# Boese0601/MagicDance

Measured on NVIDIA H100. Metric: denoise-steps/sec @512x512 50-step DDIM, higher is better.
Workload: dtype f16

## Files before the change

include/magicdance_b200.h:

```cpp
#ifndef MAGICDANCE_B200_H_
#define MAGICDANCE_B200_H_

#include <stdint.h>

#ifdef __cplusplus
extern "C" {
#endif

#define MDB_OK 0
#define MDB_ERR_INVALID (-1)
#define MDB_ERR_CUDA (-2)
#define MDB_ERR_UNSUPPORTED (-3)

#define MDB_ABI_VERSION 2

typedef void* mdb_stream_t;

int mdb_abi_version(void);
const char* mdb_last_error(void);
int mdb_device_check(void);
int64_t mdb_launch_count(void);
int64_t mdb_abi_struct_bytes(int32_t which);

#define MDB_TUNE_GEMM_PAIR_MIN_TILES 1
#define MDB_TUNE_ATTN40_2Q_MIN_CTAS 3
#define MDB_TUNE_GEMM_BN80_BELOW 4
int mdb_set_tuning(int32_t key, int32_t value);
int32_t mdb_get_tuning(int32_t key);

#define MDB_EPI_NONE 0
#define MDB_EPI_GEGLU 1

typedef struct mdb_gemm_desc {
  const void* a;
  int64_t lda;
  const void* a2;
  int64_t lda2;
  int32_t k1;
  int32_t conv;
  int32_t nb, h, w, c;
  const void* b;
  int64_t ldb;
  void* d;
  int64_t ldd;
  const float* bias;
  int64_t bias_batch_stride;
  int32_t rows_per_batch;
  int32_t epilogue;
  const void* residual;
  int64_t ldr;
  int32_t m, n, k;
  int32_t splits;
  float* splitk_ws;
  const float* ln_u;
  float ln_eps;
} mdb_gemm_desc;

int mdb_gemm_f16(const mdb_gemm_desc* desc, mdb_stream_t stream);

#define MDB_DTYPE_F16 0
#define MDB_DTYPE_F32 1

typedef struct mdb_gemm_bwd_desc {
  mdb_gemm_desc fwd;
  const void* dd; int64_t lddd;
  void* da; int64_t ldda; int32_t da_dtype; int32_t da_accumulate;
  void* da2; int64_t ldda2; int32_t da2_dtype; int32_t da2_accumulate;
  void* db; int64_t lddb; int32_t db_dtype; int32_t db_accumulate;
  float* dbias; int32_t dbias_accumulate;
  int32_t splits;
  float* ws;
} mdb_gemm_bwd_desc;

int mdb_gemm_bwd_f16(const mdb_gemm_bwd_desc* desc, mdb_stream_t stream);
int64_t mdb_gemm_bwd_ws_floats(const mdb_gemm_bwd_desc* desc);

typedef struct mdb_attn_desc {
  const void* q; int64_t ldq;
  const void* k0; int64_t ldk0; const void* vt0; int64_t ldvt0; int32_t n0; int32_t kv0_batches; int32_t ldv0_batch;
  const void* k1; int64_t ldk1; const void* vt1; int64_t ldvt1; int32_t n1; int32_t kv1_batches; int32_t ldv1_batch;
  void* out; int64_t ldo;
  int32_t batch, heads, d, nq;
  int32_t bank_batches;
  float scale;
} mdb_attn_desc;

int mdb_attention_f16(const mdb_attn_desc* desc, mdb_stream_t stream);

int mdb_attention_lse_f16(const mdb_attn_desc* desc, float* lse, mdb_stream_t stream);

typedef struct mdb_attn_bwd_desc {
  mdb_attn_desc fwd;
  const void* dout; int64_t lddout;
  const float* lse;
  void* dq; int64_t lddq;
  void* dk0; int64_t lddk0; void* dvt0; int64_t lddvt0;
  void* dk1; int64_t lddk1; void* dvt1; int64_t lddvt1;
  float* ws;
} mdb_attn_bwd_desc;

int mdb_attention_bwd_f16(const mdb_attn_bwd_desc* desc, mdb_stream_t stream);
int64_t mdb_attention_bwd_ws_floats(int32_t batch, int32_t heads, int32_t nq);

int mdb_groupnorm_f16(const void* x1, int32_t c1, const void* x2, int32_t c2, const float* gamma, const float* beta,
                      void* y, float* ws, int32_t batch, int32_t hw, float eps, int32_t silu, int32_t mode,
                      mdb_stream_t stream);
int64_t mdb_groupnorm_ws_floats(int32_t c, int32_t batch, int32_t hw);

int mdb_layernorm_f16(const void* x, const float* gamma, const float* beta, void* y, int64_t rows, int32_t c,
// ... 67 lines not shown
```

magicdance_b200/_lib.py:

```python
from __future__ import annotations

import ctypes as C
import os

from . import build as _build

c_void_p, c_int32, c_int64, c_float = C.c_void_p, C.c_int32, C.c_int64, C.c_float


class GemmDesc(C.Structure):
    _fields_ = [
        ("a", c_void_p), ("lda", c_int64), ("a2", c_void_p), ("lda2", c_int64),
        ("k1", c_int32), ("conv", c_int32), ("nb", c_int32), ("h", c_int32), ("w", c_int32), ("c", c_int32),
        ("b", c_void_p), ("ldb", c_int64), ("d", c_void_p), ("ldd", c_int64),
        ("bias", c_void_p), ("bias_batch_stride", c_int64), ("rows_per_batch", c_int32), ("epilogue", c_int32),
        ("residual", c_void_p), ("ldr", c_int64),
        ("m", c_int32), ("n", c_int32), ("k", c_int32), ("splits", c_int32), ("splitk_ws", c_void_p),
        ("ln_u", c_void_p), ("ln_eps", c_float),
    ]


class AttnDesc(C.Structure):
    _fields_ = [
        ("q", c_void_p), ("ldq", c_int64),
# ... 20 lines not shown


class GemmBwdDesc(C.Structure):
    _fields_ = [
        ("fwd", GemmDesc),
        ("dd", c_void_p), ("lddd", c_int64),
        ("da", c_void_p), ("ldda", c_int64), ("da_dtype", c_int32), ("da_accumulate", c_int32),
        ("da2", c_void_p), ("ldda2", c_int64), ("da2_dtype", c_int32), ("da2_accumulate", c_int32),
        ("db", c_void_p), ("lddb", c_int64), ("db_dtype", c_int32), ("db_accumulate", c_int32),
        ("dbias", c_void_p), ("dbias_accumulate", c_int32),
        ("splits", c_int32),
        ("ws", c_void_p),
    ]


class GroupNormBwdDesc(C.Structure):
    _fields_ = [
        ("x1", c_void_p), ("x2", c_void_p), ("c1", c_int32), ("c2", c_int32),
        ("gamma", c_void_p), ("beta", c_void_p),
        ("dy", c_void_p),
        ("batch", c_int32), ("hw", c_int32), ("eps", c_float), ("silu", c_int32),
        ("dx1", c_void_p), ("dx1_dtype", c_int32), ("dx1_accumulate", c_int32),
        ("dx2", c_void_p), ("dx2_dtype", c_int32), ("dx2_accumulate", c_int32),
        ("dgamma", c_void_p), ("dbeta", c_void_p), ("dgamma_accumulate", c_int32), ("dbeta_accumulate", c_int32),
        ("ws", c_void_p),
    ]


class LayerNormBwdDesc(C.Structure):
    _fields_ = [
        ("x", c_void_p), ("gamma", c_void_p), ("dy", c_void_p),
        ("rows", c_int64), ("c", c_int32), ("eps", c_float),
        ("dx", c_void_p), ("dx_dtype", c_int32), ("dx_accumulate", c_int32),
        ("dgamma", c_void_p), ("dbeta", c_void_p), ("dgamma_accumulate", c_int32), ("dbeta_accumulate", c_int32),
        ("ws", c_void_p),
    ]


SIGNATURES = {
    "mdb_abi_version": (c_int32, []),
    "mdb_last_error": (C.c_char_p, []),
    "mdb_device_check": (c_int32, []),
    "mdb_launch_count": (c_int64, []),
    "mdb_abi_struct_bytes": (c_int64, [c_int32]),
    "mdb_set_tuning": (c_int32, [c_int32, c_int32]),
    "mdb_get_tuning": (c_int32, [c_int32]),
    "mdb_gemm_f16": (c_int32, [C.POINTER(GemmDesc), c_void_p]),
    "mdb_gemm_bwd_f16": (c_int32, [C.POINTER(GemmBwdDesc), c_void_p]),
    "mdb_gemm_bwd_ws_floats": (c_int64, [C.POINTER(GemmBwdDesc)]),
    "mdb_attention_f16": (c_int32, [C.POINTER(AttnDesc), c_void_p]),
    "mdb_attention_lse_f16": (c_int32, [C.POINTER(AttnDesc), c_void_p, c_void_p]),
    "mdb_attention_bwd_f16": (c_int32, [C.POINTER(AttnBwdDesc), c_void_p]),
    "mdb_attention_bwd_ws_floats": (c_int64, [c_int32, c_int32, c_int32]),
    "mdb_groupnorm_f16": (c_int32, [c_void_p, c_int32, c_void_p, c_int32, c_void_p, c_void_p, c_void_p, c_void_p,
                                    c_int32, c_int32, c_float, c_int32, c_int32, c_void_p]),
    "mdb_groupnorm_ws_floats": (c_int64, [c_int32, c_int32, c_int32]),
    "mdb_layernorm_f16": (c_int32, [c_void_p, c_void_p, c_void_p, c_void_p, c_int64, c_int32, c_float, c_void_p]),
    "mdb_groupnorm_bwd_f16": (c_int32, [C.POINTER(GroupNormBwdDesc), c_void_p]),
    "mdb_groupnorm_bwd_ws_floats": (c_int64, [C.POINTER(GroupNormBwdDesc)]),
    "mdb_layernorm_bwd_f16": (c_int32, [C.POINTER(LayerNormBwdDesc), c_void_p]),
    "mdb_layernorm_bwd_ws_floats": (c_int64, [C.POINTER(LayerNormBwdDesc)]),
    "mdb_geglu_f16": (c_int32, [c_void_p, c_int64, c_void_p, c_int64, c_int64, c_int32, c_void_p]),
    "mdb_geglu_bwd_f16": (c_int32, [c_void_p, c_int64, c_void_p, c_int64, c_void_p, c_int64, c_int64, c_int32,
                                    c_void_p]),
    "mdb_conv3x3_direct_f16": (c_int32, [c_void_p, c_void_p, c_void_p, c_void_p, c_void_p, c_int32, c_int32, c_int32,
                                         c_int32, c_int32, c_int32, c_int32, c_void_p]),
    "mdb_im2col3x3_f16": (c_int32, [c_void_p, c_void_p, c_int32, c_int32, c_int32, c_int32, c_int32, c_void_p]),
    "mdb_im2col3x3_br_f16": (c_int32, [c_void_p, c_void_p, c_int32, c_int32, c_int32, c_int32, c_int32, c_void_p]),
    "mdb_upsample2x_f16": (c_int32, [c_void_p, c_void_p, c_int32, c_int32, c_int32, c_int32, c_void_p]),
    "mdb_add_f16": (c_int32, [c_void_p, c_void_p, c_void_p, c_int64, c_int32, c_int32, c_void_p]),
    "mdb_timestep_embedding_f32": (c_int32, [c_void_p, c_int32, c_void_p, c_int32, c_int32, c_void_p]),
    "mdb_skinny_linear_f32": (c_int32, [c_void_p, c_void_p, c_void_p, c_void_p, c_int32, c_int32, c_int32, c_int32,
                                        c_int32, c_void_p]),
    "mdb_nchw_f32_to_nhwc_f16": (c_int32, [c_void_p, c_void_p, c_int32, c_int32, c_int32, c_int32, c_int32, c_void_p]),
    "mdb_nhwc_f16_to_nchw_f32": (c_int32, [c_void_p, c_void_p, c_int32, c_int32, c_int32, c_int32, c_void_p]),
    "mdb_softmax_rows_f16": (c_int32, [c_void_p, c_int64, c_int32, c_int32, c_float, c_void_p]),
    "mdb_cfg_ddim_update_f32": (c_int32, [c_void_p, c_void_p, c_void_p, c_void_p, c_void_p, c_void_p, c_int64,
                                          c_void_p, c_int32, c_void_p]),
}

_lib = None
ABI_VERSION = 2
TUNE_GEMM_PAIR_MIN_TILES, TUNE_ATTN40_2Q_MIN_CTAS, TUNE_GEMM_BN80_BELOW = 1, 3, 4


def library_path() -> str:
    return os.environ.get("MAGICDANCE_B200_LIB", _build.LIB_PATH)


def load():
    global _lib
    if _lib is not None:
        return _lib
    path = library_path()
    if not os.path.isfile(path):
        raise RuntimeError(
            f"magicdance_b200: kernel library {path} is missing — run `python -m magicdance_b200.build` "
            "(there is no CPU/PyTorch fallback for the hot path)")
    if path == _build.LIB_PATH and os.path.isdir(_build.CSRC) and not _build.is_fresh():
        raise RuntimeError(f"magicdance_b200: {path} was not built from the sources in {_build.CSRC} "
                           "(stamp mismatch) — run `python -m magicdance_b200.build`")
    lib = C.CDLL(path)
    for name, (res, args) in SIGNATURES.items():
        fn = getattr(lib, name)
        fn.restype = res
        fn.argtypes = args
    if lib.mdb_abi_version() != ABI_VERSION:
        raise RuntimeError(f"magicdance_b200: ABI version mismatch ({lib.mdb_abi_version()} != {ABI_VERSION}); "
                           "rebuild the library")
    for which, mirror in ((0, GemmDesc), (1, AttnDesc), (2, AttnBwdDesc), (3, GemmBwdDesc), (4, GroupNormBwdDesc),
                          (5, LayerNormBwdDesc)):
        if lib.mdb_abi_struct_bytes(which) != C.sizeof(mirror):
            raise RuntimeError(f"magicdance_b200: {mirror.__name__} mirrors {C.sizeof(mirror)} bytes, the library's "
                               f"struct has {lib.mdb_abi_struct_bytes(which)}: the binding and the library disagree")
    _lib = lib
    return lib


def check(rc: int, what: str):
    if rc != 0:
        msg = load().mdb_last_error().decode(errors="replace")
        raise RuntimeError(f"magicdance_b200.{what} failed (code {rc}): {msg}")
```

magicdance_b200/csrc/attention.cu:

```cuda
#include <stdlib.h>

#include <type_traits>

#include "common.cuh"

namespace mdb {

constexpr int kBQ = 128;

template <int D, int BKV, int STAGES>
struct AttnCfg {
  static constexpr int kDkChunks = (D + 63) / 64;
  static constexpr int kDV = (D + 15) / 16 * 16;
  static constexpr int kKSteps = kDV / 16;
  static constexpr int kQBytes = kDkChunks * kBQ * 128;
  static constexpr int kKBytes = kDkChunks * BKV * 128;
  static constexpr int kVBytes = kDV * 128;
  static constexpr int kStageBytes = kKBytes + kVBytes;
  static constexpr int kSmem = kQBytes + STAGES * kStageBytes + 1024;
  static_assert(BKV == 64, "one 128-byte swizzle row of keys per V^T tile");
  static_assert(kVBytes % 1024 == 0 && kKBytes % 1024 == 0, "stage tiles start on swizzle-atom boundaries");
};

struct AttnKParams {
// ... 92 lines not shown
      }
      wgmma_commit();
      wgmma_wait<0>();
      wgmma_fence_regs(sc);

      if (valid < BKV) {
#pragma unroll
        for (int i = 0; i < BKV / 2; ++i)
          if (8 * (i >> 2) + cq + (i & 1) >= valid) sc[i] = -INFINITY;
      }
      float mx[2] = {-INFINITY, -INFINITY};
#pragma unroll
      for (int i = 0; i < BKV / 2; ++i) mx[(i >> 1) & 1] = fmaxf(mx[(i >> 1) & 1], sc[i]);
      float alpha[2], neg_m[2];
#pragma unroll
      for (int h = 0; h < 2; ++h) {
        mx[h] = fmaxf(mx[h], __shfl_xor_sync(0xffffffffu, mx[h], 1));
        mx[h] = fmaxf(mx[h], __shfl_xor_sync(0xffffffffu, mx[h], 2));
        const float m_new = fmaxf(m_run[h], mx[h] * p.scale_log2);
        alpha[h] = ex2_approx(m_run[h] - m_new);
        m_run[h] = m_new;
        neg_m[h] = -m_new;
      }
      float ls[2] = {0.f, 0.f};
      uint32_t pa[BKV / 16][4];
#pragma unroll
      for (int i = 0; i < BKV / 2; i += 2) {
        const int h = (i >> 1) & 1;
        const float e0 = ex2_approx(fmaf(sc[i], p.scale_log2, neg_m[h]));
        const float e1 = ex2_approx(fmaf(sc[i + 1], p.scale_log2, neg_m[h]));
        ls[h] += e0 + e1;
        pa[i >> 3][(i >> 1) & 3] = pack_half2(e0, e1);
      }
#pragma unroll
      for (int h = 0; h < 2; ++h) l_run[h] = fmaf(l_run[h], alpha[h], ls[h]);
#pragma unroll
      for (int i = 0; i < C::kDV / 2; ++i) o[i] *= alpha[(i >> 1) & 1];

      wgmma_fence();
#pragma unroll
      for (int kk = 0; kk < BKV / 16; ++kk)
        wgmma_rs<C::kDV>(o, pa[kk], wgmma_desc_k_sw128(v_addr) + 2 * kk, 1u);
      wgmma_commit();
      wgmma_wait<0>();
      wgmma_fence_regs(o);
      mbar_arrive(&kv_empty[s]);
    }

    float inv_l[2], l_row[2];
#pragma unroll
    for (int h = 0; h < 2; ++h) {
      float l = l_run[h];
      l += __shfl_xor_sync(0xffffffffu, l, 1);
      l += __shfl_xor_sync(0xffffffffu, l, 2);
      inv_l[h] = 1.0f / l;
      l_row[h] = l;
    }
    const int r = wg * 64 + (warp & 3) * 16 + (lane >> 2);
    if constexpr (LSE) {
      if ((lane & 3) == 0) {
#pragma unroll
        for (int h = 0; h < 2; ++h) {
          const int q = q0 + r + 8 * h;
          if (q < p.nq)
            p.lse[(static_cast<long long>(b) * gridDim.y + head) * p.nq + q] =
                (m_run[h] + log2f(l_row[h])) * 0.6931471805599453f;
        }
      }
    }
#pragma unroll
    for (int h = 0; h < 2; ++h) {
      const int q = q0 + r + 8 * h;
      if (q < p.nq) {
        __half* op = p.out + (static_cast<long long>(b) * p.nq + q) * p.ldo + head * D + cq;
#pragma unroll
        for (int c8 = 0; c8 < D / 8; ++c8)
          *reinterpret_cast<uint32_t*>(op + 8 * c8) =
              pack_half2(o[4 * c8 + 2 * h] * inv_l[h], o[4 * c8 + 2 * h + 1] * inv_l[h]);
      }
    }
  }
}

static int g_attn40_2q_min_ctas = 512;
int get_attn_tuning() { return g_attn40_2q_min_ctas; }
void set_attn_tuning(int v) { g_attn40_2q_min_ctas = v; }

template <int D, int BKV, int STAGES, int MINB, bool LSE = false, typename P>
static int launch_attn(const P& kp, dim3 grid, cudaStream_t st) {
  using C = AttnCfg<D, BKV, STAGES>;
  static_assert(MINB == 1 || C::kSmem <= 113 * 1024, "two CTAs per SM must fit");
  constexpr auto kern = attn_wg_kernel<D, BKV, STAGES, MINB, LSE>;
  if (int rc = set_max_dyn_smem<kern>(C::kSmem)) return rc;
  MDB_CHECK_CUDA(launch_pdl(kern, grid, dim3(kWsThreads), C::kSmem, st, kp));
  count_launch();
  return MDB_OK;
}

template <int D, int BKV>
static int build_and_launch(const mdb_attn_desc* a, float* lse, cudaStream_t st) {
  constexpr int kDV = AttnCfg<D, BKV, 1>::kDV;
  AttnKParams kp;
  memset(&kp, 0, sizeof(kp));
  const int hd = a->heads * a->d;
  int rc;
  if ((rc = tmap_heads(&kp.tmQ, a->q, a->d, a->heads, (uint64_t)a->batch * a->nq, a->ldq, kBQ))) return rc;
  auto mk_kv = [&](const void* k, long long ldk, const void* vt, long long ldvt, int n, int nb, int ldvb,
                   CUtensorMap* tk, CUtensorMap* tv) -> int {
    int r = tmap_heads(tk, k, a->d, a->heads, (uint64_t)nb * n, ldk, BKV);
    if (r) return r;
    return tmap_vt(tv, vt, n, nb, ldvb, hd, ldvt, kDV);
  };
  if ((rc = mk_kv(a->k0, a->ldk0, a->vt0, a->ldvt0, a->n0, a->kv0_batches, a->ldv0_batch, &kp.tmK0, &kp.tmV0))) return rc;
  if (a->n1 > 0) {
    if ((rc = mk_kv(a->k1, a->ldk1, a->vt1, a->ldvt1, a->n1, a->kv1_batches, a->ldv1_batch, &kp.tmK1, &kp.tmV1)))
      return rc;
  }
  kp.out = static_cast<__half*>(a->out);
  kp.ldo = a->ldo;
  kp.nq = a->nq;
  kp.n0 = a->n0;
  kp.n1 = a->n1;
  kp.kv0_batches = a->kv0_batches;
  kp.kv1_batches = a->kv1_batches;
  kp.bank_batches = a->n1 > 0 ? a->bank_batches : 0;
  kp.scale_log2 = a->scale * 1.4426950408889634f;
  dim3 grid((a->nq + kBQ - 1) / kBQ, a->heads, a->batch);
  if (lse != nullptr) {
    AttnLseKParams lp;
    memset(&lp, 0, sizeof(lp));
    static_cast<AttnKParams&>(lp) = kp;
    lp.lse = lse;
    if constexpr (D == 40) {
      const long long ctas = (long long)grid.x * grid.y * grid.z;
      if (ctas >= (long long)g_attn40_2q_min_ctas) return launch_attn<D, BKV, 3, 2, true>(lp, grid, st);
    }
    return launch_attn<D, BKV, (D == 160 ? 2 : 4), 1, true>(lp, grid, st);
  }
  if constexpr (D == 40) {
    const long long ctas = (long long)grid.x * grid.y * grid.z;
    if (ctas >= (long long)g_attn40_2q_min_ctas) return launch_attn<D, BKV, 3, 2>(kp, grid, st);
  }
  return launch_attn<D, BKV, (D == 160 ? 2 : 4), 1>(kp, grid, st);
}

static int attention_entry(const mdb_attn_desc* a, float* lse, cudaStream_t st) {
  switch (a->d) {
    case 40:
      return build_and_launch<40, 64>(a, lse, st);
    case 80:
      return build_and_launch<80, 64>(a, lse, st);
    case 160:
      return build_and_launch<160, 64>(a, lse, st);
    default:
      set_error("mdb_attention_f16: head dim %d not supported (40, 80, 160)", a->d);
      return MDB_ERR_UNSUPPORTED;
  }
}

int attention_check_desc(const mdb_attn_desc* a) {
  MDB_REQUIRE(a != nullptr, "mdb_attention_f16: null descriptor");
  MDB_REQUIRE(a->q && a->k0 && a->vt0 && a->out, "mdb_attention_f16: null operand");
  MDB_REQUIRE(a->batch > 0 && a->heads > 0 && a->nq > 0 && a->n0 > 0 && a->n1 >= 0,
              "mdb_attention_f16: bad shape");
  MDB_REQUIRE(a->n1 == 0 || (a->k1 && a->vt1), "mdb_attention_f16: n1 > 0 needs k1/vt1");
  MDB_REQUIRE(a->kv0_batches == 1 || a->kv0_batches == a->batch, "mdb_attention_f16: kv0_batches must be 1 or batch");
  MDB_REQUIRE(a->n1 == 0 || a->kv1_batches == 1 || a->kv1_batches >= a->bank_batches,
              "mdb_attention_f16: kv1_batches must be 1 or cover bank_batches");
  MDB_REQUIRE(a->ldv0_batch >= a->n0 && a->ldv0_batch % 8 == 0, "mdb_attention_f16: ldv0_batch must be >= n0 and %% 8");
  MDB_REQUIRE(a->n1 == 0 || (a->ldv1_batch >= a->n1 && a->ldv1_batch % 8 == 0),
              "mdb_attention_f16: ldv1_batch must be >= n1 and %% 8");
  MDB_REQUIRE(a->ldo % 8 == 0 && (reinterpret_cast<uintptr_t>(a->out) & 15) == 0, "mdb_attention_f16: out alignment");
  return MDB_OK;
}

}

using namespace mdb;

extern "C" int mdb_attention_f16(const mdb_attn_desc* a, mdb_stream_t stream) {
  const int rc = attention_check_desc(a);
  if (rc) return rc;
  return attention_entry(a, nullptr, static_cast<cudaStream_t>(stream));
}

extern "C" int mdb_attention_lse_f16(const mdb_attn_desc* a, float* lse, mdb_stream_t stream) {
  const int rc = attention_check_desc(a);
  if (rc) return rc;
  MDB_REQUIRE(lse != nullptr, "mdb_attention_lse_f16: null lse");
  return attention_entry(a, lse, static_cast<cudaStream_t>(stream));
}
```

magicdance_b200/csrc/common.cuh:

```cuda
#pragma once

#include <cuda.h>
#include <cuda_fp16.h>
#include <cuda_runtime.h>
#include <cudaTypedefs.h>
#include <stdint.h>
#include <stdio.h>
#include <string.h>

#include "../../include/magicdance_b200.h"
#include "wgmma.cuh"

namespace mdb {

void set_error(const char* fmt, ...);

#define MDB_CHECK_CUDA(expr)                                                                     \
  do {                                                                                           \
    cudaError_t _e = (expr);                                                                     \
    if (_e != cudaSuccess) {                                                                     \
      mdb::set_error("%s:%d: %s failed: %s", __FILE__, __LINE__, #expr, cudaGetErrorString(_e)); \
      return MDB_ERR_CUDA;                                                                       \
    }                                                                                            \
  } while (0)

#define MDB_REQUIRE(cond, ...)      \
  do {                              \
    if (!(cond)) {                  \
      mdb::set_error(__VA_ARGS__);  \
      return MDB_ERR_INVALID;       \
    }                               \
  } while (0)

void count_launch(int n = 1);
int get_gemm_tuning(int key);
void set_gemm_tuning(int key, int value);
int get_attn_tuning();
void set_attn_tuning(int v);

constexpr int kNumSms = 132;

int tmap_rows(CUtensorMap* out, const void* base, uint64_t inner, uint64_t rows, long long ld, uint32_t box_inner,
              uint32_t box_rows);
int tmap_heads(CUtensorMap* out, const void* base, int d, int heads, uint64_t tokens, long long ld,
               uint32_t box_tokens);
int tmap_vt(CUtensorMap* out, const void* base, int n, int nb, long long ldvb, int rows, long long ldvt,
            uint32_t box_rows);
int tmap_nhwc(CUtensorMap* out, const void* base, int c, int w, int h, int nb, long long ld, const uint32_t box[4],
              int cs);

enum { kBoxOk, kBoxWideRows, kBoxRowsPerTile, kBoxImagesPerTile, kBoxTooLarge };
int pixel_box(int ho, int wo, int cs, int rows, bool fwd, uint32_t box[4]);

#ifdef __CUDACC__

bool pdl_enabled();
template <typename... KArgs, typename... Args>
inline cudaError_t launch_pdl_cluster2(void (*kernel)(KArgs...), dim3 grid, dim3 block, size_t smem,
                                       cudaStream_t stream, unsigned cluster_x, unsigned cluster_z, Args&&... args) {
  cudaLaunchConfig_t cfg;
  memset(&cfg, 0, sizeof(cfg));
  cfg.gridDim = grid;
  cfg.blockDim = block;
  cfg.dynamicSmemBytes = smem;
  cfg.stream = stream;
  cudaLaunchAttribute attr[2];
  int n = 0;
  if (cluster_z > 1 || cluster_x > 1) {
    attr[n].id = cudaLaunchAttributeClusterDimension;
    attr[n].val.clusterDim.x = cluster_x;
    attr[n].val.clusterDim.y = 1;
    attr[n].val.clusterDim.z = cluster_z;
    ++n;
  }
  if (pdl_enabled()) {
    attr[n].id = cudaLaunchAttributeProgrammaticStreamSerialization;
    attr[n].val.programmaticStreamSerializationAllowed = 1;
    ++n;
  }
  cfg.attrs = attr;
  cfg.numAttrs = n;
  return cudaLaunchKernelEx(&cfg, kernel, static_cast<KArgs>(args)...);
}
template <typename... KArgs, typename... Args>
inline cudaError_t launch_pdl_cluster(void (*kernel)(KArgs...), dim3 grid, dim3 block, size_t smem,
                                      cudaStream_t stream, unsigned cluster_z, Args&&... args) {
  return launch_pdl_cluster2(kernel, grid, block, smem, stream, 1u, cluster_z, static_cast<Args&&>(args)...);
}
template <typename... KArgs, typename... Args>
inline cudaError_t launch_pdl(void (*kernel)(KArgs...), dim3 grid, dim3 block, size_t smem, cudaStream_t stream,
                              Args&&... args) {
  return launch_pdl_cluster2(kernel, grid, block, smem, stream, 1u, 1u, static_cast<Args&&>(args)...);
}
template <auto Kernel>
inline int set_max_dyn_smem(int bytes) {
  static bool done = false;
  if (!done) {
    MDB_CHECK_CUDA(cudaFuncSetAttribute(Kernel, cudaFuncAttributeMaxDynamicSharedMemorySize, bytes));
    done = true;
  }
  return MDB_OK;
}

__device__ __forceinline__ uint32_t smem_u32(const void* p) {
  return static_cast<uint32_t>(__cvta_generic_to_shared(p));
}

__device__ __forceinline__ bool elect_one() {
  uint32_t pred = 0;
  asm volatile(
      "{\n\t.reg .pred P;\n\t"
      "elect.sync _|P, 0xffffffff;\n\t"
      "selp.u32 %0, 1, 0, P;\n\t}"
      : "=r"(pred));
  return pred != 0;
}

__device__ __forceinline__ void pdl_launch_dependents() { asm volatile("griddepcontrol.launch_dependents;" ::: "memory"); }
__device__ __forceinline__ void pdl_wait() { asm volatile("griddepcontrol.wait;" ::: "memory"); }

__device__ __forceinline__ void mbar_init(uint64_t* bar, uint32_t count) {
// ... 48 lines not shown
  const int s = it % S;
  mbar_wait(&full[s], (it / S) & 1);
  return s;
}

__device__ __forceinline__ void tma_prefetch_desc(const CUtensorMap* m) {
  asm volatile("prefetch.tensormap [%0];" ::"l"(reinterpret_cast<uint64_t>(m)) : "memory");
}
__device__ __forceinline__ void tma_load_2d(void* dst, const CUtensorMap* m, uint64_t* bar, int c0, int c1) {
  asm volatile(
      "cp.async.bulk.tensor.2d.shared::cluster.global.tile.mbarrier::complete_tx::bytes [%0], [%1, {%3, %4}], [%2];"
      ::"r"(smem_u32(dst)), "l"(reinterpret_cast<uint64_t>(m)), "r"(smem_u32(bar)), "r"(c0), "r"(c1)
      : "memory");
}
__device__ __forceinline__ void tma_load_3d(void* dst, const CUtensorMap* m, uint64_t* bar, int c0, int c1, int c2) {
  asm volatile(
      "cp.async.bulk.tensor.3d.shared::cluster.global.tile.mbarrier::complete_tx::bytes [%0], [%1, {%3, %4, %5}], [%2];"
      ::"r"(smem_u32(dst)), "l"(reinterpret_cast<uint64_t>(m)), "r"(smem_u32(bar)), "r"(c0), "r"(c1), "r"(c2)
      : "memory");
}
__device__ __forceinline__ void tma_load_4d(void* dst, const CUtensorMap* m, uint64_t* bar, int c0, int c1, int c2,
                                            int c3) {
  asm volatile(
      "cp.async.bulk.tensor.4d.shared::cluster.global.tile.mbarrier::complete_tx::bytes [%0], [%1, {%3, %4, %5, %6}], [%2];"
      ::"r"(smem_u32(dst)), "l"(reinterpret_cast<uint64_t>(m)), "r"(smem_u32(bar)), "r"(c0), "r"(c1), "r"(c2), "r"(c3)
      : "memory");
}

__device__ __forceinline__ uint32_t cluster_ctarank() {
  uint32_t r;
  asm volatile("mov.u32 %0, %%cluster_ctarank;" : "=r"(r));
  return r;
}
__device__ __forceinline__ void cluster_sync_all() {
  asm volatile("barrier.cluster.arrive.release.aligned;" ::: "memory");
  asm volatile("barrier.cluster.wait.acquire.aligned;" ::: "memory");
}
__device__ __forceinline__ uint32_t dsmem_map(uint32_t local_smem_addr, uint32_t rank) {
  uint32_t a;
  asm volatile("mapa.shared::cluster.u32 %0, %1, %2;" : "=r"(a) : "r"(local_smem_addr), "r"(rank));
  return a;
}
__device__ __forceinline__ float4 dsmem_ld_f4(uint32_t cluster_addr) {
  float4 v;
  asm volatile("ld.shared::cluster.v4.f32 {%0, %1, %2, %3}, [%4];"
               : "=f"(v.x), "=f"(v.y), "=f"(v.z), "=f"(v.w)
               : "r"(cluster_addr));
  return v;
}

__device__ __forceinline__ void fence_proxy_async_smem() {
  asm volatile("fence.proxy.async.shared::cta;" ::: "memory");
}

__device__ __forceinline__ uint64_t wgmma_desc_k_sw128(uint32_t smem_addr) {
  uint64_t d = 0;
  d |= static_cast<uint64_t>((smem_addr & 0x3FFFF) >> 4);
  d |= static_cast<uint64_t>(1) << 16;
  d |= static_cast<uint64_t>(1024 >> 4) << 32;
  d |= static_cast<uint64_t>(1) << 62;
  return d;
}
__device__ __forceinline__ uint64_t wgmma_desc_mn_sw128(uint32_t smem_addr, uint32_t chunk_bytes) {
  uint64_t d = 0;
  d |= static_cast<uint64_t>((smem_addr & 0x3FFFF) >> 4);
  d |= static_cast<uint64_t>((chunk_bytes >> 4) & 0x3FFF) << 16;
  d |= static_cast<uint64_t>(1024 >> 4) << 32;
  d |= static_cast<uint64_t>(1) << 62;
  return d;
}
__device__ __forceinline__ void wgmma_fence() { asm volatile("wgmma.fence.sync.aligned;" ::: "memory"); }
__device__ __forceinline__ void wgmma_commit() { asm volatile("wgmma.commit_group.sync.aligned;" ::: "memory"); }
template <int N>
__device__ __forceinline__ void wgmma_wait() { asm volatile("wgmma.wait_group.sync.aligned %0;" ::"n"(N) : "memory"); }
template <int R>
__device__ __forceinline__ void wgmma_fence_regs(float (&d)[R]) {
#pragma unroll
  for (int i = 0; i < R; ++i) asm volatile("" : "+f"(d[i])::"memory");
}
__device__ __forceinline__ void named_bar_sync(int id, int threads) {
  asm volatile("bar.sync %0, %1;" ::"r"(id), "r"(threads) : "memory");
}

__device__ __forceinline__ uint32_t pack_half2(float a, float b) {
  __half2 h = __floats2half2_rn(a, b);
  return *reinterpret_cast<uint32_t*>(&h);
}

__device__ __forceinline__ float ex2_approx(float x) {
  float y;
  asm("ex2.approx.ftz.f32 %0, %1;" : "=f"(y) : "f"(x));
  return y;
}
__device__ __forceinline__ float silu_f(float x) { return x / (1.0f + __expf(-x)); }
__device__ __forceinline__ float gelu_erf_f(float x) { return 0.5f * x * (1.0f + erff(x * 0.70710678118654752f)); }
__device__ __forceinline__ float dsilu(float x) {
  const float s = 1.0f / (1.0f + __expf(-x));
  return s * (1.0f + x * (1.0f - s));
}
__device__ __forceinline__ float dgelu_erf(float x) {
  return 0.5f * (1.0f + erff(x * 0.70710678118654752f)) + x * 0.39894228040143268f * __expf(-0.5f * x * x);
}

struct GbOut {
  void* p;
  long long ld;
  int f32, acc;
};

__device__ __forceinline__ void gb_store2(const GbOut& o, long long row, int col, float v0, float v1) {
  if (o.p == nullptr) return;
  if (o.f32) {
    float2* d = reinterpret_cast<float2*>(static_cast<float*>(o.p) + row * o.ld + col);
    if (o.acc) {
      const float2 x = *d;
      v0 += x.x;
      v1 += x.y;
    }
    *d = make_float2(v0, v1);
  } else {
    __half2* d = reinterpret_cast<__half2*>(static_cast<__half*>(o.p) + row * o.ld + col);
    if (o.acc) {
      const float2 x = __half22float2(*d);
      v0 += x.x;
      v1 += x.y;
    }
    *d = __floats2half2_rn(v0, v1);
  }
}
#endif

inline GbOut gb_out(void* p, long long ld, int dtype, int acc) {
  GbOut o;
  o.p = p;
  o.ld = ld;
  o.f32 = dtype == MDB_DTYPE_F32;
  o.acc = acc != 0;
  return o;
}

int launch_colsum_finalize(const float* ws, int n, int segs, int parts, float* out, long long stride, int acc,
                           cudaStream_t st);

}
```

magicdance_b200/csrc/misc.cu:

```cuda
#include <stdarg.h>
#include <stdlib.h>

#include <atomic>

#include "common.cuh"

namespace mdb {

static thread_local char g_err[512] = "";
static std::atomic<long long> g_launches{0};

void set_error(const char* fmt, ...) {
  va_list ap;
  va_start(ap, fmt);
  vsnprintf(g_err, sizeof(g_err), fmt, ap);
  va_end(ap);
}
void count_launch(int n) { g_launches.fetch_add(n, std::memory_order_relaxed); }
bool pdl_enabled() { return true; }

static PFN_cuTensorMapEncodeTiled_v12000 g_encode = nullptr;

static int make_tmap_f16(CUtensorMap* out, const void* base, int rank, const uint64_t* dims,
                         const uint64_t* strides_bytes, const uint32_t* box, const uint32_t* elem_strides = nullptr) {
// ... 434 lines not shown
    const int b = static_cast<int>(r / (static_cast<long long>(w) * h)) % batch;
    y[i] = __float2half_rn(x[((static_cast<long long>(b) * c + ch) * h + yy) * w + xx]);
  }
}

__global__ void nhwc_f16_to_nchw_f32_kernel(const __half* __restrict__ x, float* __restrict__ y, int batch, int c, int h,
                                            int w) {
  pdl_launch_dependents();
  pdl_wait();
  const long long total = static_cast<long long>(batch) * c * h * w;
  for (long long i = static_cast<long long>(blockIdx.x) * blockDim.x + threadIdx.x; i < total;
       i += static_cast<long long>(gridDim.x) * blockDim.x) {
    const int xx = static_cast<int>(i % w);
    long long r = i / w;
    const int yy = static_cast<int>(r % h);
    r /= h;
    const int ch = static_cast<int>(r % c);
    const int b = static_cast<int>(r / c);
    y[i] = __half2float(x[((static_cast<long long>(b) * h + yy) * w + xx) * c + ch]);
  }
}

__global__ void cfg_ddim_update_kernel(float* x, const float* __restrict__ ec, const float* __restrict__ eu,
                                       const float* __restrict__ noise, float* __restrict__ x_prev,
                                       float* __restrict__ pred_x0, long long n, const float* __restrict__ coef,
                                       int update_x) {
  pdl_launch_dependents();
  pdl_wait();
  const float scale = coef[0], sqrt_at = coef[1], sqrt_aprev = coef[2], dir_coef = coef[3], sigma = coef[4],
              s1m = coef[5];
  for (long long i = static_cast<long long>(blockIdx.x) * blockDim.x + threadIdx.x; i < n;
       i += static_cast<long long>(gridDim.x) * blockDim.x) {
    const float u = eu[i];
    const float e = u + scale * (ec[i] - u);
    const float p0 = (x[i] - s1m * e) / sqrt_at;
    float xp = sqrt_aprev * p0 + dir_coef * e;
    if (noise != nullptr) xp += sigma * noise[i];
    x_prev[i] = xp;
    pred_x0[i] = p0;
    if (update_x) x[i] = xp;
  }
}


static inline int grid_for(long long total, int threads = 256, int cap = kNumSms * 16) {
  long long b = (total + threads - 1) / threads;
  if (b > cap) b = cap;
  if (b < 1) b = 1;
  return static_cast<int>(b);
}

}

using namespace mdb;

extern "C" int mdb_abi_version(void) { return MDB_ABI_VERSION; }

extern "C" int64_t mdb_abi_struct_bytes(int32_t which) {
  switch (which) {
    case 0:
      return (int64_t)sizeof(mdb_gemm_desc);
    case 1:
      return (int64_t)sizeof(mdb_attn_desc);
    case 2:
      return (int64_t)sizeof(mdb_attn_bwd_desc);
    case 3:
      return (int64_t)sizeof(mdb_gemm_bwd_desc);
    case 4:
      return (int64_t)sizeof(mdb_groupnorm_bwd_desc);
    case 5:
      return (int64_t)sizeof(mdb_layernorm_bwd_desc);
    default:
      return -1;
  }
}

extern "C" int mdb_set_tuning(int32_t key, int32_t value) {
  switch (key) {
    case MDB_TUNE_GEMM_PAIR_MIN_TILES:
    case MDB_TUNE_GEMM_BN80_BELOW:
      mdb::set_gemm_tuning(key, value);
      return MDB_OK;
    case MDB_TUNE_ATTN40_2Q_MIN_CTAS:
      mdb::set_attn_tuning(value);
      return MDB_OK;
    default:
      mdb::set_error("mdb_set_tuning: unknown key %d", key);
      return MDB_ERR_INVALID;
  }
}

extern "C" int32_t mdb_get_tuning(int32_t key) {
  if (key == MDB_TUNE_ATTN40_2Q_MIN_CTAS) return mdb::get_attn_tuning();
  return mdb::get_gemm_tuning(key);
}
extern "C" const char* mdb_last_error(void) { return mdb::g_err; }
extern "C" int64_t mdb_launch_count(void) { return mdb::g_launches.load(); }

extern "C" int mdb_device_check(void) {
  int dev = 0;
  MDB_CHECK_CUDA(cudaGetDevice(&dev));
  cudaDeviceProp prop;
  MDB_CHECK_CUDA(cudaGetDeviceProperties(&prop, dev));
  if (prop.major != 9 || prop.minor != 0) {
    set_error("device %d is sm_%d%d; this library is built for sm_90a only", dev, prop.major, prop.minor);
    return MDB_ERR_UNSUPPORTED;
  }
  return MDB_OK;
}

namespace {
__global__ void __launch_bounds__(256) softmax_rows_kernel(__half* __restrict__ x, long long ld, int cols, float scale_log2) {
  mdb::pdl_launch_dependents();
  mdb::pdl_wait();
  __shared__ float red[8];
  __shared__ float bcast;
  __half* row = x + static_cast<long long>(blockIdx.x) * ld;
  const int vecs = cols >> 3;
  const int lane = threadIdx.x & 31, warp = threadIdx.x >> 5;
  float m = -INFINITY;
  for (int v = threadIdx.x; v < vecs; v += blockDim.x) {
    const uint4 u = *reinterpret_cast<const uint4*>(row + v * 8);
    const __half2* h2 = reinterpret_cast<const __half2*>(&u);
#pragma unroll
    for (int e = 0; e < 4; ++e) {
      const float2 f = __half22float2(h2[e]);
      m = fmaxf(m, fmaxf(f.x, f.y));
    }
  }
#pragma unroll
  for (int o = 16; o > 0; o >>= 1) m = fmaxf(m, __shfl_xor_sync(0xffffffffu, m, o));
  if (lane == 0) red[warp] = m;
  __syncthreads();
  if (threadIdx.x == 0) {
    float t = red[0];
    for (int w = 1; w < 8; ++w) t = fmaxf(t, red[w]);
    bcast = t;
  }
  __syncthreads();
  m = bcast * scale_log2;
  float sum = 0.f;
  for (int v = threadIdx.x; v < vecs; v += blockDim.x) {
    const uint4 u = *reinterpret_cast<const uint4*>(row + v * 8);
    const __half2* h2 = reinterpret_cast<const __half2*>(&u);
#pragma unroll
    for (int e = 0; e < 4; ++e) {
      const float2 f = __half22float2(h2[e]);
      sum += exp2f(fmaf(f.x, scale_log2, -m)) + exp2f(fmaf(f.y, scale_log2, -m));
    }
  }
#pragma unroll
  for (int o = 16; o > 0; o >>= 1) sum += __shfl_xor_sync(0xffffffffu, sum, o);
  __syncthreads();
  if (lane == 0) red[warp] = sum;
  __syncthreads();
  if (threadIdx.x == 0) {
    float t = 0.f;
    for (int w = 0; w < 8; ++w) t += red[w];
    bcast = 1.0f / t;
  }
  __syncthreads();
  const float inv = bcast;
  for (int v = threadIdx.x; v < vecs; v += blockDim.x) {
    uint4 u = *reinterpret_cast<const uint4*>(row + v * 8);
    __half2* h2 = reinterpret_cast<__half2*>(&u);
#pragma unroll
    for (int e = 0; e < 4; ++e) {
      const float2 f = __half22float2(h2[e]);
      h2[e] = __floats2half2_rn(exp2f(fmaf(f.x, scale_log2, -m)) * inv, exp2f(fmaf(f.y, scale_log2, -m)) * inv);
    }
    *reinterpret_cast<uint4*>(row + v * 8) = u;
  }
}
}

extern "C" int mdb_softmax_rows_f16(void* x, int64_t ld, int32_t rows, int32_t cols, float scale, mdb_stream_t stream) {
// ... 163 lines not shown
```

magicdance_b200/ops.py:

```python
from __future__ import annotations

import ctypes as C
import os

import torch

from . import _lib

EPI_NONE, EPI_GEGLU = 0, 1
SKINNY_MAX_ROWS = 16
_GEMM_DEBUG = os.environ.get("MDB_GEMM_DEBUG", "0") == "1"
TRACE = None


class tuning:
    _KEYS = {"pair_min_tiles": _lib.TUNE_GEMM_PAIR_MIN_TILES,
             "attn40_2q_min_ctas": _lib.TUNE_ATTN40_2Q_MIN_CTAS, "bn80_below": _lib.TUNE_GEMM_BN80_BELOW}

    def __init__(self, **kw):
        self.want = {self._KEYS[k]: int(v) for k, v in kw.items() if v is not None}

    def __enter__(self):
        lib = _lib.load()
        self.old = {k: int(lib.mdb_get_tuning(k)) for k in self.want}
        for k, v in self.want.items():
            _lib.check(lib.mdb_set_tuning(k, v), "set_tuning")
        return self

    def __exit__(self, *a):
        lib = _lib.load()
        for k, v in self.old.items():
            lib.mdb_set_tuning(k, v)


def _stream() -> int:
    return torch.cuda.current_stream().cuda_stream


def _ptr(t):
    return None if t is None else t.data_ptr()


def _chk(t: torch.Tensor, dtype, name):
    if not t.is_cuda:
        raise RuntimeError(f"magicdance_b200: {name} must be a CUDA tensor (no CPU fallback exists for the hot path)")
    if t.dtype != dtype:
        raise RuntimeError(f"magicdance_b200: {name} must be {dtype}, got {t.dtype}")


def require_cuda(device):
    if torch.device(device).type != "cuda":
        raise RuntimeError("magicdance_b200: the networks run only on an sm_90 CUDA device — move the model to "
                           "the GPU first (there is no CPU/PyTorch fallback for the hot path)")


def ensure_device():
    lib = _lib.load()
    if not torch.cuda.is_available():
        raise RuntimeError("magicdance_b200: no CUDA device visible; the hot path has no CPU fallback")
    _lib.check(lib.mdb_device_check(), "device_check")
    return lib


def launch_count() -> int:
    return int(_lib.load().mdb_launch_count())


_ws_cache = {}


_ws_tag = 0


class workspace_lane:

    def __init__(self, tag):
        self.tag = tag

    def __enter__(self):
        global _ws_tag
        self.prev, _ws_tag = _ws_tag, self.tag

    def __exit__(self, *a):
        global _ws_tag
        _ws_tag = self.prev


def current_lane():
    return _ws_tag


_ws_retired = []


def _workspace(key, numel, dtype, device, zero=False):
    k = (key, device, _ws_tag)
    t = _ws_cache.get(k)
    if t is None or t.numel() < numel or t.dtype != dtype:
        if t is not None:
            _ws_retired.append(t)
# ... 624 lines not shown
```

Baseline: 89.98.

## Add warp-specialized pipelined head-dim-40 attention kernel for long key sequences

```diff
diff --git a/include/magicdance_b200.h b/include/magicdance_b200.h
--- a/include/magicdance_b200.h
+++ b/include/magicdance_b200.h
@@ -25,6 +25,9 @@
 #define MDB_TUNE_GEMM_PAIR_MIN_TILES 1
 #define MDB_TUNE_ATTN40_2Q_MIN_CTAS 3
 #define MDB_TUNE_GEMM_BN80_BELOW 4
+enum {
+  MDB_TUNE_ATTN40_PIPE_MIN_KEYS = 5
+};
 int mdb_set_tuning(int32_t key, int32_t value);
 int32_t mdb_get_tuning(int32_t key);
 
diff --git a/magicdance_b200/_lib.py b/magicdance_b200/_lib.py
--- a/magicdance_b200/_lib.py
+++ b/magicdance_b200/_lib.py
@@ -126,6 +126,7 @@
 _lib = None
 ABI_VERSION = 2
 TUNE_GEMM_PAIR_MIN_TILES, TUNE_ATTN40_2Q_MIN_CTAS, TUNE_GEMM_BN80_BELOW = 1, 3, 4
+TUNE_ATTN40_PIPE_MIN_KEYS = 5
 
 
 def library_path() -> str:
diff --git a/magicdance_b200/csrc/attention.cu b/magicdance_b200/csrc/attention.cu
--- a/magicdance_b200/csrc/attention.cu
+++ b/magicdance_b200/csrc/attention.cu
@@ -198,9 +198,228 @@
   }
 }
 
+constexpr int kBKV40 = 128;
+constexpr int kStages40 = 4;
+struct Attn40PipeCfg {
+  static constexpr int kDV = 48;
+  static constexpr int kKSteps = kDV / 16;
+  static constexpr int kQBytes = kBQ * 128;
+  static constexpr int kKBytes = kBKV40 * 128;
+  static constexpr int kVChunkBytes = kDV * 128;
+  static constexpr int kStageBytes = kKBytes + 2 * kVChunkBytes;
+  static constexpr int kSmem = kQBytes + kStages40 * kStageBytes + 1024;
+  static_assert(kVChunkBytes % 1024 == 0 && kKBytes % 1024 == 0, "stage tiles start on swizzle-atom boundaries");
+};
+
+constexpr int kPipeThreads = kConsumers + 128;
+template <bool LSE>
+__global__ void __launch_bounds__(kPipeThreads, 1)
+    attn40_pipe_kernel(const __grid_constant__ std::conditional_t<LSE, AttnLseKParams, AttnKParams> p) {
+  using C = Attn40PipeCfg;
+  constexpr int D = 40, BKV = kBKV40, STAGES = kStages40;
+  extern __shared__ uint8_t smem_raw[];
+  __shared__ __align__(8) uint64_t q_bar;
+  __shared__ __align__(8) uint64_t kv_full[STAGES], kv_empty[STAGES];
+
+  uint8_t* sQ = align1024(smem_raw);
+  uint8_t* sKV = sQ + C::kQBytes;
+
+  const int warp = threadIdx.x >> 5;
+  const int lane = threadIdx.x & 31;
+  const int q0 = blockIdx.x * kBQ;
+  const int head = blockIdx.y;
+  const int b = blockIdx.z;
+  const int t0 = (p.n0 + BKV - 1) / BKV;
+  const int t1 = (b < p.bank_batches && p.n1 > 0) ? (p.n1 + BKV - 1) / BKV : 0;
+  const int n_tiles = t0 + t1;
+
+  pdl_launch_dependents();
+  if (warp == kProducerWarp && lane == 0) {
+    tma_prefetch_desc(&p.tmQ);
+    tma_prefetch_desc(&p.tmK0);
+    tma_prefetch_desc(&p.tmV0);
+    mbar_init(&q_bar, 1);
+    ring_init<STAGES>(kv_full, kv_empty, 1);
+    fence_barrier_init();
+  }
+  __syncthreads();
+  pdl_wait();
+
+  if (warp >= kProducerWarp) {
+    setmaxnreg_dec<40>();
+    if (warp == kProducerWarp && lane == 0) {
+      mbar_expect_tx(&q_bar, C::kQBytes);
+      tma_load_3d(sQ, &p.tmQ, &q_bar, 0, head, b * p.nq + q0);
+      for (int j = 0; j < n_tiles; ++j) {
+        const bool src1 = j >= t0;
+        const int key0 = (src1 ? (j - t0) : j) * BKV;
+        const CUtensorMap* tk = src1 ? &p.tmK1 : &p.tmK0;
+        const CUtensorMap* tv = src1 ? &p.tmV1 : &p.tmV0;
+        const int nsrc = src1 ? p.n1 : p.n0;
+        const int kvb = src1 ? (p.kv1_batches > 1 ? b : 0) : (p.kv0_batches > 1 ? b : 0);
+        const bool two = nsrc - key0 > 64;
+        const int s = ring_acquire<STAGES>(kv_empty, j);
+        mbar_expect_tx(&kv_full[s], C::kKBytes + (two ? 2 : 1) * C::kVChunkBytes);
+        uint8_t* sk = sKV + s * C::kStageBytes;
+        uint8_t* sv = sk + C::kKBytes;
+        tma_load_3d(sk, tk, &kv_full[s], 0, head, kvb * nsrc + key0);
+        tma_load_3d(sv, tv, &kv_full[s], key0, kvb, head * D);
+        if (two) tma_load_3d(sv + C::kVChunkBytes, tv, &kv_full[s], key0 + 64, kvb, head * D);
+      }
+    }
+  } else {
+    setmaxnreg_inc<232>();
+    const int wg = warp >> 2;
+    const uint32_t q_addr = smem_u32(sQ) + wg * (64 * 128);
+    const int cq = 2 * (lane & 3);
+    float o[C::kDV / 2];
+#pragma unroll
+    for (int i = 0; i < C::kDV / 2; ++i) o[i] = 0.f;
+    float m_run[2] = {-INFINITY, -INFINITY};
+    float l_run[2] = {0.f, 0.f};
+    float sc[BKV / 2];
+    uint32_t pa0[BKV / 16][4], pa1[BKV / 16][4];
+    mbar_wait(&q_bar, 0);
+
+    auto issue_qk = [&](int s) {
+      const uint32_t k_addr = smem_u32(sKV + s * C::kStageBytes);
+#pragma unroll
+      for (int ks = 0; ks < C::kKSteps; ++ks)
+        wgmma_ss<BKV>(sc, wgmma_desc_k_sw128(q_addr) + 2 * ks, wgmma_desc_k_sw128(k_addr) + 2 * ks, ks != 0 ? 1u : 0u);
+    };
+    auto tile_keys = [&](int j) { return j >= t0 ? min(BKV, p.n1 - (j - t0) * BKV) : min(BKV, p.n0 - j * BKV); };
+    auto issue_pv = [&](int s, const uint32_t (&pa)[BKV / 16][4], int keys) {
+      const uint32_t v_addr = smem_u32(sKV + s * C::kStageBytes) + C::kKBytes;
+#pragma unroll
+      for (int kk = 0; kk < 4; ++kk) wgmma_rs<C::kDV>(o, pa[kk], wgmma_desc_k_sw128(v_addr) + 2 * kk, 1u);
+      if (keys > 64) {
+#pragma unroll
+        for (int kk = 4; kk < 8; ++kk)
+          wgmma_rs<C::kDV>(o, pa[kk], wgmma_desc_k_sw128(v_addr + C::kVChunkBytes) + 2 * (kk - 4), 1u);
+      }
+    };
+    auto softmax = [&](int j, float (&alpha)[2], uint32_t (&pn)[BKV / 16][4]) {
+      const int valid = tile_keys(j);
+      if (valid < BKV) {
+#pragma unroll
+        for (int i = 0; i < BKV / 2; ++i)
+          if (8 * (i >> 2) + cq + (i & 1) >= valid) sc[i] = -INFINITY;
+      }
+      float mx[2] = {-INFINITY, -INFINITY};
+#pragma unroll
+      for (int i = 0; i < BKV / 2; ++i) mx[(i >> 1) & 1] = fmaxf(mx[(i >> 1) & 1], sc[i]);
+      float neg_m[2];
+#pragma unroll
+      for (int h = 0; h < 2; ++h) {
+        mx[h] = fmaxf(mx[h], __shfl_xor_sync(0xffffffffu, mx[h], 1));
+        mx[h] = fmaxf(mx[h], __shfl_xor_sync(0xffffffffu, mx[h], 2));
+        const float m_new = fmaxf(m_run[h], mx[h] * p.scale_log2);
+        alpha[h] = ex2_approx(m_run[h] - m_new);
+        m_run[h] = m_new;
+        neg_m[h] = -m_new;
+      }
+      float ls[2] = {0.f, 0.f};
+#pragma unroll
+      for (int i = 0; i < BKV / 2; i += 2) {
+        const int h = (i >> 1) & 1;
+        const float e0 = ex2_approx(fmaf(sc[i], p.scale_log2, neg_m[h]));
+        const float e1 = ex2_approx(fmaf(sc[i + 1], p.scale_log2, neg_m[h]));
+        ls[h] += e0 + e1;
+        pn[i >> 3][(i >> 1) & 3] = pack_half2(e0, e1);
+      }
+#pragma unroll
+      for (int h = 0; h < 2; ++h) l_run[h] = fmaf(l_run[h], alpha[h], ls[h]);
+    };
+
+    int s_prev = 0;
+    auto step = [&](int j, const uint32_t (&p_prev)[BKV / 16][4], uint32_t (&p_new)[BKV / 16][4]) {
+      const int s = ring_wait_full<STAGES>(kv_full, j);
+      wgmma_fence();
+      issue_qk(s);
+      wgmma_commit();
+      issue_pv(s_prev, p_prev, tile_keys(j - 1));
+      wgmma_commit();
+      wgmma_wait<1>();
+      wgmma_fence_regs(sc);
+      float alpha[2];
+      softmax(j, alpha, p_new);
+      wgmma_wait<0>();
+      wgmma_fence_regs(o);
+      mbar_arrive(&kv_empty[s_prev]);
+#pragma unroll
+      for (int i = 0; i < C::kDV / 2; ++i) o[i] *= alpha[(i >> 1) & 1];
+      s_prev = s;
+    };
+    {
+      s_prev = ring_wait_full<STAGES>(kv_full, 0);
+      wgmma_fence();
+      issue_qk(s_prev);
+      wgmma_commit();
+      wgmma_wait<0>();
+      wgmma_fence_regs(sc);
+      float alpha[2];
+      softmax(0, alpha, pa0);
+    }
+    for (int j = 1; j < n_tiles; j += 2) {
+      step(j, pa0, pa1);
+      if (j + 1 < n_tiles) step(j + 1, pa1, pa0);
+    }
+    wgmma_fence();
+    if (n_tiles & 1)
+      issue_pv(s_prev, pa0, tile_keys(n_tiles - 1));
+    else
+      issue_pv(s_prev, pa1, tile_keys(n_tiles - 1));
+    wgmma_commit();
+    wgmma_wait<0>();
+    wgmma_fence_regs(o);
+    mbar_arrive(&kv_empty[s_prev]);
+
+    float inv_l[2], l_row[2];
+#pragma unroll
+    for (int h = 0; h < 2; ++h) {
+      float l = l_run[h];
+      l += __shfl_xor_sync(0xffffffffu, l, 1);
+      l += __shfl_xor_sync(0xffffffffu, l, 2);
+      inv_l[h] = 1.0f / l;
+      l_row[h] = l;
+    }
+    const int r = wg * 64 + (warp & 3) * 16 + (lane >> 2);
+    if constexpr (LSE) {
+      if ((lane & 3) == 0) {
+#pragma unroll
+        for (int h = 0; h < 2; ++h) {
+          const int q = q0 + r + 8 * h;
+          if (q < p.nq)
+            p.lse[(static_cast<long long>(b) * gridDim.y + head) * p.nq + q] =
+                (m_run[h] + log2f(l_row[h])) * 0.6931471805599453f;
+        }
+      }
+    }
+#pragma unroll
+    for (int h = 0; h < 2; ++h) {
+      const int q = q0 + r + 8 * h;
+      if (q < p.nq) {
+        __half* op = p.out + (static_cast<long long>(b) * p.nq + q) * p.ldo + head * D + cq;
+#pragma unroll
+        for (int c8 = 0; c8 < D / 8; ++c8)
+          *reinterpret_cast<uint32_t*>(op + 8 * c8) =
+              pack_half2(o[4 * c8 + 2 * h] * inv_l[h], o[4 * c8 + 2 * h + 1] * inv_l[h]);
+      }
+    }
+  }
+}
+
 static int g_attn40_2q_min_ctas = 512;
-int get_attn_tuning() { return g_attn40_2q_min_ctas; }
-void set_attn_tuning(int v) { g_attn40_2q_min_ctas = v; }
+static int g_attn40_pipe_min_keys = 256;
+int get_attn_tuning(int key) {
+  return key == MDB_TUNE_ATTN40_2Q_MIN_CTAS ? g_attn40_2q_min_ctas : g_attn40_pipe_min_keys;
+}
+void set_attn_tuning(int key, int v) {
+  if (key == MDB_TUNE_ATTN40_2Q_MIN_CTAS)
+    g_attn40_2q_min_ctas = v;
+  else
+    g_attn40_pipe_min_keys = v;
+}
 
 template <int D, int BKV, int STAGES, int MINB, bool LSE = false, typename P>
 static int launch_attn(const P& kp, dim3 grid, cudaStream_t st) {
@@ -213,9 +432,19 @@
   return MDB_OK;
 }
 
+template <bool LSE, typename P>
+static int launch_attn40_pipe(const P& kp, dim3 grid, cudaStream_t st) {
+  constexpr auto kern = attn40_pipe_kernel<LSE>;
+  if (int rc = set_max_dyn_smem<kern>(Attn40PipeCfg::kSmem)) return rc;
+  MDB_CHECK_CUDA(launch_pdl(kern, grid, dim3(kPipeThreads), Attn40PipeCfg::kSmem, st, kp));
+  count_launch();
+  return MDB_OK;
+}
+
 template <int D, int BKV>
 static int build_and_launch(const mdb_attn_desc* a, float* lse, cudaStream_t st) {
   constexpr int kDV = AttnCfg<D, BKV, 1>::kDV;
+  const bool pipe = D == 40 && (long long)a->n0 + a->n1 >= g_attn40_pipe_min_keys;
   AttnKParams kp;
   memset(&kp, 0, sizeof(kp));
   const int hd = a->heads * a->d;
@@ -223,7 +452,7 @@
   if ((rc = tmap_heads(&kp.tmQ, a->q, a->d, a->heads, (uint64_t)a->batch * a->nq, a->ldq, kBQ))) return rc;
   auto mk_kv = [&](const void* k, long long ldk, const void* vt, long long ldvt, int n, int nb, int ldvb,
                    CUtensorMap* tk, CUtensorMap* tv) -> int {
-    int r = tmap_heads(tk, k, a->d, a->heads, (uint64_t)nb * n, ldk, BKV);
+    int r = tmap_heads(tk, k, a->d, a->heads, (uint64_t)nb * n, ldk, pipe ? kBKV40 : BKV);
     if (r) return r;
     return tmap_vt(tv, vt, n, nb, ldvb, hd, ldvt, kDV);
   };
@@ -248,12 +477,14 @@
     static_cast<AttnKParams&>(lp) = kp;
     lp.lse = lse;
     if constexpr (D == 40) {
+      if (pipe) return launch_attn40_pipe<true>(lp, grid, st);
       const long long ctas = (long long)grid.x * grid.y * grid.z;
       if (ctas >= (long long)g_attn40_2q_min_ctas) return launch_attn<D, BKV, 3, 2, true>(lp, grid, st);
     }
     return launch_attn<D, BKV, (D == 160 ? 2 : 4), 1, true>(lp, grid, st);
   }
   if constexpr (D == 40) {
+    if (pipe) return launch_attn40_pipe<false>(kp, grid, st);
     const long long ctas = (long long)grid.x * grid.y * grid.z;
     if (ctas >= (long long)g_attn40_2q_min_ctas) return launch_attn<D, BKV, 3, 2>(kp, grid, st);
   }
diff --git a/magicdance_b200/csrc/common.cuh b/magicdance_b200/csrc/common.cuh
--- a/magicdance_b200/csrc/common.cuh
+++ b/magicdance_b200/csrc/common.cuh
@@ -35,8 +35,8 @@
 void count_launch(int n = 1);
 int get_gemm_tuning(int key);
 void set_gemm_tuning(int key, int value);
-int get_attn_tuning();
-void set_attn_tuning(int v);
+int get_attn_tuning(int key);
+void set_attn_tuning(int key, int value);
 
 constexpr int kNumSms = 132;
 
@@ -251,6 +251,11 @@
   asm volatile("bar.sync %0, %1;" ::"r"(id), "r"(threads) : "memory");
 }
 
+template <int N>
+__device__ __forceinline__ void setmaxnreg_dec() { asm volatile("setmaxnreg.dec.sync.aligned.u32 %0;" ::"n"(N)); }
+template <int N>
+__device__ __forceinline__ void setmaxnreg_inc() { asm volatile("setmaxnreg.inc.sync.aligned.u32 %0;" ::"n"(N)); }
+
 __device__ __forceinline__ uint32_t pack_half2(float a, float b) {
   __half2 h = __floats2half2_rn(a, b);
   return *reinterpret_cast<uint32_t*>(&h);
diff --git a/magicdance_b200/csrc/misc.cu b/magicdance_b200/csrc/misc.cu
--- a/magicdance_b200/csrc/misc.cu
+++ b/magicdance_b200/csrc/misc.cu
@@ -540,7 +540,8 @@
       mdb::set_gemm_tuning(key, value);
       return MDB_OK;
     case MDB_TUNE_ATTN40_2Q_MIN_CTAS:
-      mdb::set_attn_tuning(value);
+    case MDB_TUNE_ATTN40_PIPE_MIN_KEYS:
+      mdb::set_attn_tuning(key, value);
       return MDB_OK;
     default:
       mdb::set_error("mdb_set_tuning: unknown key %d", key);
@@ -549,7 +550,7 @@
 }
 
 extern "C" int32_t mdb_get_tuning(int32_t key) {
-  if (key == MDB_TUNE_ATTN40_2Q_MIN_CTAS) return mdb::get_attn_tuning();
+  if (key == MDB_TUNE_ATTN40_2Q_MIN_CTAS || key == MDB_TUNE_ATTN40_PIPE_MIN_KEYS) return mdb::get_attn_tuning(key);
   return mdb::get_gemm_tuning(key);
 }
 extern "C" const char* mdb_last_error(void) { return mdb::g_err; }
diff --git a/magicdance_b200/ops.py b/magicdance_b200/ops.py
--- a/magicdance_b200/ops.py
+++ b/magicdance_b200/ops.py
@@ -15,7 +15,8 @@
 
 class tuning:
     _KEYS = {"pair_min_tiles": _lib.TUNE_GEMM_PAIR_MIN_TILES,
-             "attn40_2q_min_ctas": _lib.TUNE_ATTN40_2Q_MIN_CTAS, "bn80_below": _lib.TUNE_GEMM_BN80_BELOW}
+             "attn40_2q_min_ctas": _lib.TUNE_ATTN40_2Q_MIN_CTAS, "bn80_below": _lib.TUNE_GEMM_BN80_BELOW,
+             "attn40_pipe_min_keys": _lib.TUNE_ATTN40_PIPE_MIN_KEYS}
 
     def __init__(self, **kw):
         self.want = {self._KEYS[k]: int(v) for k, v in kw.items() if v is not None}
```

Result: no change. 90.55, median of 6 (+0.6%).
